# DecodeGenetics/BamQC

Measured on AMD Instinct MI355X. Metric: BAM records/sec (and GB/s vs HBM roofline), 150 bp PE, 1/2/4/8 MI355X, higher is better.
Workload: dtype u8/u32/u64 integer

## Files before the change

### bamqc_amd/csrc/k_short.hip

```cpp
#include "kernels_common.h"
#include "read_stats.h"
#include "swar.h"

#define KS_NH BQC_FAST_NH
#define KS_NB (8 * KS_NH)
#define KS_ND (2 * KS_NH)
#define KS_CSTRIDE (256 / KS_NB)
#define KS_LUTW (KS_NH == 2 ? 8 : 16)
#define KS_WAVES BQC_FAST_WAVES
#define KS_THREADS (KS_WAVES * 64)
#define KS_CT 256
#define KS_T8    0
#define KS_TRIP  (KS_T8 + 16384)
#define KS_CYC   (KS_TRIP + 1024)
#define KS_NC    (KS_CYC + 2 * 6 * KS_CT)
#define KS_GC    (KS_NC + 2 * (KS_CT + 1))
#define KS_AQ    (KS_GC + 2 * (KS_CT + 1))
#define KS_AC    (KS_AQ + 512)
#define KS_LUT   (KS_AC + 512)
#define KS_META  (KS_LUT + (KS_NB + 1) * KS_LUTW + (((KS_NB + 1) * KS_LUTW) % 4 ? 4 - ((KS_NB + 1) * KS_LUTW) % 4 : 0))
#define KS_MW    8
#define KS_RS    (KS_META + (KS_WAVES * 64 + 1) * KS_MW)
#define KS_WORDS (KS_RS + RS_WORDS)
#define KS_T8_PERIOD 16
#define KS_BIAS  512u

static_assert((KS_LUT % 4) == 0 && (KS_META % 4) == 0, "16-byte alignment of the LDS tables");

__device__ __forceinline__ bool t8_flush(uint32_t* lds, uint64_t* __restrict__ em, uint4* __restrict__ slot , uint32_t n_rows_used)
{
    if (slot && n_rows_used < BQC_T8_SPW) {
        uint4* row = slot + (size_t)n_rows_used * 4096u;
        uint4* src = (uint4*)(lds + KS_T8);
        for (uint32_t i = threadIdx.x; i < 4096u; i += blockDim.x) { row[i] = src[i]; src[i] = make_uint4(0, 0, 0, 0); }
        return true;
    }
    t8_atomics_out(lds + KS_T8, em);
    return false;
}

__device__ __forceinline__ uint32_t ks_trip_bin(uint32_t ix) { return ix ^ ((ix >> 2) & 0x11u); }
__device__ __forceinline__ uint32_t ks_trip_stream(uint32_t s) { return s ^ ((s >> 2) & 0x11111111u); }

__device__ __forceinline__ bool ks_flush(uint32_t* lds, const StateLayout& sl, uint64_t* __restrict__ state, uint32_t lane, uint4* __restrict__ slot, uint32_t n_rows_used)
{
    const uint64_t lb = sl.lane_base(lane);
    const bool wrote_row = t8_flush(lds, state + lb + sl.o_eightmer, slot, n_rows_used);
    for (uint32_t i = threadIdx.x; i < 1024; i += blockDim.x) {
        const uint32_t v = lds[KS_TRIP + i];
        if (!v) continue;
        lds[KS_TRIP + i] = 0;
        const uint32_t ix = ks_trip_bin(i);
        const uint32_t grp = i >> 8, f3 = (ix >> 6) & 3u, f2 = (ix >> 4) & 3u, f1 = (ix >> 2) & 3u, f0 = ix & 3u;
        uint32_t ctx, base;
        if (grp < 2u) { ctx = (f3 << 4) | (f2 << 2) | f0; base = f1; }
        else { ctx = ((3u - f0) << 4) | ((3u - f2) << 2) | (3u - f3); base = 3u - f1; }
        gadd(state + lb + sl.o_triplet + ctx * 16u + grp * 4u + base, v);
    }
    for (uint32_t i = threadIdx.x; i < 2 * 6 * KS_CT; i += blockDim.x) {
        const uint32_t v = lds[KS_CYC + i];
        if (!v) continue;
        lds[KS_CYC + i] = 0;
        const uint32_t m = i / (6 * KS_CT), c = (i / KS_CT) % 6, jj = i % KS_CT, j = (jj % KS_CSTRIDE) * KS_NB + jj / KS_CSTRIDE;
        if (j < sl.lcap) gadd(state + sl.mate_base(lane, m) + (c < 5 ? sl.m_dnacount + c * sl.lcap : sl.m_qualcount) + j, v);
    }
    for (uint32_t i = threadIdx.x; i < 2 * (KS_CT + 1); i += blockDim.x) {
        const uint32_t m = i / (KS_CT + 1), j = i % (KS_CT + 1);
        const uint64_t mb = sl.mate_base(lane, m);
        uint32_t v = lds[KS_NC + i];
        if (v && j <= sl.lcap) gadd(state + mb + sl.m_ncount + j, v);
        lds[KS_NC + i] = 0;
        v = lds[KS_GC + i];
        if (v && j <= sl.lcap) gadd(state + mb + sl.m_gccount + j, v);
        lds[KS_GC + i] = 0;
    }
    for (uint32_t i = threadIdx.x; i < 512; i += blockDim.x) {
        const uint64_t mb = sl.mate_base(lane, i >> 8);
        uint32_t v = lds[KS_AQ + i];
        if (v) gadd(state + mb + sl.m_avgqual + (i & 255), v);
        lds[KS_AQ + i] = 0;
        v = lds[KS_AC + i];
        if (v) gadd(state + mb + sl.m_avgceil + (i & 255), v);
        lds[KS_AC + i] = 0;
    }
    return wrote_row;
}

struct CycAcc {
    uint32_t l1[KS_NH][4];
    uint32_t qo[KS_ND], qe[KS_ND];
};
__device__ __forceinline__ void cyc_zero(CycAcc& A)
{
#pragma unroll
    for (int h = 0; h < KS_NH; ++h)
#pragma unroll
        for (int p = 0; p < 4; ++p) A.l1[h][p] = 0;
#pragma unroll
    for (int d = 0; d < KS_ND; ++d) { A.qo[d] = 0; A.qe[d] = 0; }
}
__device__ __noinline__ void cyc_spill_half(uint32_t a, uint32_t c, uint32_t g, uint32_t t, uint32_t* base )
{
    const uint32_t v[4] = {a, c, g, t};
#pragma unroll
    for (int p = 0; p < 4; ++p)
#pragma unroll
        for (int n = 0; n < 8; ++n) atomicAdd(base + p * KS_CT + KS_CSTRIDE * (7 - n), (v[p] >> (4 * n)) & 15u);
}
__device__ __noinline__ void cyc_qflush_pair(uint32_t o0, uint32_t e0, uint32_t o1, uint32_t e1, uint32_t* base )
{
    const uint32_t vo[2] = {o0, o1}, ve[2] = {e0, e1};
#pragma unroll
    for (int d = 0; d < 2; ++d) {
        atomicAdd(base + KS_CSTRIDE * (4 * d + 0), vo[d] >> 16);
        atomicAdd(base + KS_CSTRIDE * (4 * d + 1), ve[d] >> 16);
        atomicAdd(base + KS_CSTRIDE * (4 * d + 2), vo[d] & 0xFFFFu);
        atomicAdd(base + KS_CSTRIDE * (4 * d + 3), ve[d] & 0xFFFFu);
    }
}
__device__ __forceinline__ void cyc_spill(CycAcc& A, uint32_t* lds, uint32_t mate, uint32_t w)
{
#pragma unroll
    for (int h = 0; h < KS_NH; ++h) {
        cyc_spill_half(A.l1[h][0], A.l1[h][1], A.l1[h][2], A.l1[h][3], lds + KS_CYC + mate * 6 * KS_CT + w + KS_CSTRIDE * 8 * h);
#pragma unroll
        for (int p = 0; p < 4; ++p) A.l1[h][p] = 0;
    }
}
__device__ __forceinline__ void cyc_qflush(CycAcc& A, uint32_t* lds, uint32_t mate, uint32_t w)
{
#pragma unroll
    for (int h = 0; h < KS_NH; ++h) {
        cyc_qflush_pair(A.qo[2 * h], A.qe[2 * h], A.qo[2 * h + 1], A.qe[2 * h + 1], lds + KS_CYC + (mate * 6 + 5) * KS_CT + w + KS_CSTRIDE * 8 * h);
        A.qo[2 * h] = A.qe[2 * h] = A.qo[2 * h + 1] = A.qe[2 * h + 1] = 0;
    }
}
__device__ __forceinline__ void cyc_add(CycAcc& A, const Planes (&P)[KS_NH], const uint32_t (&Q)[KS_ND])
{
#pragma unroll
    for (int h = 0; h < KS_NH; ++h) { A.l1[h][0] += P[h].a; A.l1[h][1] += P[h].c; A.l1[h][2] += P[h].g; A.l1[h][3] += P[h].t; }
#pragma unroll
    for (int d = 0; d < KS_ND; ++d) { A.qe[d] += Q[d] & 0x00FF00FFu; A.qo[d] += __builtin_amdgcn_perm(0u, Q[d], 0x0C030C01u); }
}

#define KM_PRIM   0x10000u
#define KM_TRIP   0x20000u
#define KM_SEG    0x40000u

__device__ __forceinline__ void lut_nib(uint32_t (&d)[KS_NH], const uint32_t* e)
{
    if (KS_NH == 2) { const uint2 v = *(const uint2*)e; d[0] = v.x; d[1] = v.y; }
    else { const uint4 v = *(const uint4*)e; d[0] = v.x; d[1] = v.y; d[KS_NH - 2] = v.z; d[KS_NH - 1] = v.w; }
}
__device__ __forceinline__ void lut_byte(uint32_t (&d)[KS_ND], const uint32_t* e)
{
#pragma unroll
    for (int q = 0; q < KS_ND / 4; ++q) { const uint4 v = *(const uint4*)(e + 4 * q); d[4 * q] = v.x; d[4 * q + 1] = v.y; d[4 * q + 2] = v.z; d[4 * q + 3] = v.w; }
}

template <bool S> struct KsTile { static constexpr bool seg = S; };

struct Pre { uint32_t s[KS_NH + 1], q[KS_ND], e[KS_NH + 1]; uint32_t m0, pp, w5; };

__device__ __forceinline__ Pre ks_prefetch(const uint32_t* rec, uint32_t w, const uint8_t* seqb, const uint8_t* qualb)
{
    const uint4 ma = *(const uint4*)rec, mb = *(const uint4*)(rec + 4);
    const int32_t sw = (ma.x & 0x10u) ? -(int32_t)w : (int32_t)w;
    Pre P;
    P.m0 = ma.x;
    P.w5 = mb.y;
    P.pp = ma.w + (uint32_t)(KS_NB * sw);
    GVec<KS_NH + 1>::ldu(P.s, seqb + (uint32_t)(ma.y + (uint32_t)(KS_NB / 2 * sw)));
    GVec<KS_ND>::ldu(P.q, qualb + (uint32_t)(ma.z + (uint32_t)(KS_NB * sw)));
    const uint32_t* rn = (const uint32_t*)(uintptr_t)((uint64_t)mb.z | ((uint64_t)mb.w << 32));
    const int32_t di = min(max((int32_t)P.pp >> 3, 0), (int32_t)mb.x);
    GVec<KS_NH + 1>::lda(P.e, (const uint8_t*)(rn + di));
    return P;
}

__global__ __launch_bounds__(KS_THREADS) void k_short(DevBatch b, StateLayout sl, uint64_t* __restrict__ state, DevRefs refs,
                                                         uint32_t* __restrict__ err, uint32_t parts, uint4* __restrict__ t8rows,
                                                         uint32_t* __restrict__ t8_used, uint32_t t8_period)
{
    extern __shared__ uint32_t lds[];
    if ((uint32_t)(uintptr_t)(lds_u32*)lds != 0u) {
        if (threadIdx.x == 0) { atomicOr(err, BQC_DEVERR_INTERNAL); t8_used[blockIdx.x * BQC_T8_USED] = 0; }
        return;
    }
    for (uint32_t i = threadIdx.x; i < KS_WORDS; i += blockDim.x) lds[i] = 0;
    block_sync();
    const uint32_t M = 0x11111111u;
    const uint32_t ln = threadIdx.x & 63u, wave = (uint32_t)__builtin_amdgcn_readfirstlane((int)(threadIdx.x >> 6));
    const BatchDesc desc = *b.desc;
    const uint32_t W = desc.fast_w, rpw = 64u / W;
    const uint32_t slot = ln / W, w = ln % W, wnb = KS_NB * w;
    const bool lane_used = slot < rpw;
    const bool last_w = (w + 1u >= W) || ln == 63u;
    const uint32_t tile_cap = rpw * (64u / rpw);
    uint32_t* WM = lds + KS_META + wave * 64u * KS_MW;
    const uint32_t* DUMMY = lds + KS_META + KS_WAVES * 64u * KS_MW;
    const uint32_t* LUT = lds + KS_LUT;
    if (threadIdx.x <= KS_NB) {
        const uint32_t n = threadIdx.x;
        uint32_t* e = lds + KS_LUT + KS_LUTW * n;
        for (uint32_t h = 0; h < KS_NH; ++h) {
            const uint32_t v = n > 8u * h ? (n - 8u * h < 8u ? n - 8u * h : 8u) : 0u;
            e[h] = v ? 0xFFFFFFFFu << (4u * (8u - v)) : 0u;
        }
        for (uint32_t d = 0; d < KS_ND; ++d) {
            const uint32_t v = n > 4u * d ? (n - 4u * d < 4u ? n - 4u * d : 4u) : 0u;
            e[4 + d] = v ? 0xFFFFFFFFu << (8u * (4u - v)) : 0u;
        }
    }
    if (threadIdx.x < KS_MW) {
        const uint32_t t = threadIdx.x;
        lds[KS_META + KS_WAVES * 64u * KS_MW + t] = t == 1 || t == 2 ? KS_BIAS : t == 3 ? 8u * KS_NH - 1u : t == 5 ? (24u << 16) : t == 6 ? (uint32_t)(uintptr_t)state
                                   : t == 7 ? (uint32_t)((uintptr_t)state >> 32) : 0u;
    }
    block_sync();
    CycAcc A;
    cyc_zero(A);
    const uint32_t mate = slot < (rpw + 1u) / 2u ? 0u : 1u;
    uint32_t n1 = 0, n2 = 0;
    uint32_t cur_lane = 0xFFFFFFFFu, since_t8 = 0;
    uint4* const t8_slot = t8rows + (size_t)blockIdx.x * BQC_T8_SPW * 4096u;
    uint32_t t8_n = 0;
    T8Tags t8_tags;

    const uint8_t* g_seq = b.seq - KS_BIAS;
    const uint8_t* g_qual = b.qual - KS_BIAS;
    const uint32_t n_chunks = desc.n_chunks_fast;
    {
        const uint32_t cpw = (n_chunks + gridDim.x - 1) / gridDim.x;
        t8_period = max(t8_period, (cpw + BQC_T8_SPW - 2) / (BQC_T8_SPW - 1));
    }
    uint32_t ci = blockIdx.x, ci_step = gridDim.x, ci_end = n_chunks;
    if ((parts & 16u) && (gridDim.x & 7u) == 0u && n_chunks >= gridDim.x) {
        const uint32_t per = (n_chunks + 7u) >> 3, lo = (blockIdx.x & 7u) * per;
        ci = lo + (blockIdx.x >> 3); ci_step = gridDim.x >> 3; ci_end = min(n_chunks, lo + per);
    }
    for (;; ci += ci_step) {
        const bool done = ci >= ci_end;
        Chunk ch{0, 0, 0xFFFFFFFFu, 0, 0, 0, 0, 0};
        if (!done) ch = b.chunks_fast[ci];
        if (ch.lane != cur_lane) {
            if (cur_lane != 0xFFFFFFFFu) {
                if (lane_used) { cyc_spill(A, lds, mate, w); cyc_qflush(A, lds, mate, w); }
                n1 = n2 = 0;
                block_sync();
                if (ks_flush(lds, sl, state, cur_lane, t8_slot, t8_n)) { t8_tag(t8_tags, t8_n, cur_lane); ++t8_n; }
                rs_flush(lds + KS_RS, sl, state, cur_lane);
            }
            cur_lane = ch.lane;
            since_t8 = 0;
        }
        if (done) break;
        if (++since_t8 > t8_period) {
            since_t8 = 1;
            const bool to_row = t8_n < BQC_T8_SPW;
            uint32_t* row = (uint32_t*)(t8_slot + (size_t)t8_n * 4096u);
            uint64_t* emf = state + sl.lane_base(cur_lane) + sl.o_eightmer;
#pragma unroll 4
            for (uint32_t k = 0; k < 16384u / (KS_WAVES * 64u); ++k) {
                const uint32_t i = (wave * (16384u / (KS_WAVES * 64u)) + k) * 64u + ln;
                const uint32_t v = atomicExch(&lds[KS_T8 + i], 0u);
                if (to_row) row[i] = v;
                else if (v) {
#pragma unroll
                    for (uint32_t b8 = 0; b8 < 4; ++b8)
                        if ((v >> (8u * b8)) & 0xFFu) gadd(emf + 4u * i + ((4u - b8) & 3u), (v >> (8u * b8)) & 0xFFu);
                }
            }
            if (to_row) { t8_tag(t8_tags, t8_n, cur_lane); ++t8_n; }
        }
        const uint64_t lb = sl.lane_base(cur_lane);
        uint64_t* em = state + lb + sl.o_eightmer;
        const uint32_t n_seg = ch.count - ch.aux;
        const uint32_t my_tiles = ch.aux > wave * tile_cap ? (ch.aux - wave * tile_cap + KS_WAVES * tile_cap - 1u) / (KS_WAVES * tile_cap) : 0u;
        const uint32_t sw0 = (wave + KS_WAVES - ci % KS_WAVES) % KS_WAVES;
        const uint32_t seg_tiles = n_seg > sw0 * tile_cap ? (n_seg - sw0 * tile_cap + KS_WAVES * tile_cap - 1u) / (KS_WAVES * tile_cap) : 0u;
        for (uint32_t tix = 0; tix < my_tiles + seg_tiles; ++tix) {
        const bool seg_tile = tix >= my_tiles;
        const uint32_t tb = seg_tile ? (sw0 + (tix - my_tiles) * KS_WAVES) * tile_cap : (wave + tix * KS_WAVES) * tile_cap;
        const uint32_t p_first = seg_tile ? ch.aux : 0u, p_n = seg_tile ? n_seg : ch.aux;
        const uint32_t tn = min(tile_cap, p_n - tb);
        __builtin_amdgcn_s_setprio(3);
        uint32_t r;
        bool stat;
        {
            const uint32_t t = ch.first + p_first + tb + ln;
            r = ln < tn ? b.perm[t] : 0xFFFFFFFFu;
            const bool live = r != 0xFFFFFFFFu;
            const bool seg = live && (r & BQC_ENTRY_SEG);
            stat = live && !seg;
            TripSeg sg{0, 0, 0, 0};
            if (seg) { sg = b.segs[r & ~BQC_ENTRY_SEG]; r = sg.r; }
            uint4 R0 = make_uint4(0u, KS_BIAS, KS_BIAS, 8u * KS_NH - 1u);
            uint4 R1 = make_uint4(0u, 24u << 16, (uint32_t)(uintptr_t)state, (uint32_t)((uintptr_t)state >> 32));
            if (live) {
                const uint32_t fl = b.flag[r];
                R0.x = fl & 0xFFFFu;
                if (!(fl & 0x900u) && (fl & 0xC0u)) {
                    const uint32_t L = b.l_seq[r];
                    const bool rc = fl & 0x10u, noq = fl & BQC_FLAG_NO_QUAL;
                    const int32_t o0 = rc ? (int32_t)L - KS_NB : 0;
                    R0.x |= (seg ? KM_SEG : KM_PRIM) | (L << 20);
                    R0.y = b.seq_off[r] + (uint32_t)((o0 - 1) >> 1) + KS_BIAS;
                    R0.z = (noq ? 0u : b.qual_off[r]) + (uint32_t)o0 + KS_BIAS;
                    R1.y = ((o0 & 1) ? 28u : 24u) << 16;
                    const int32_t rid = b.rid[r];
                    if ((fl & BQC_FLAG_TRIPLET) && b.n_cigar[r] >= 1 && L >= 3 && !noq && rid >= 0 && (uint32_t)rid < refs.n_refs &&
                        refs.refn[rid] != nullptr) {
                        const int64_t pos = seg ? (int64_t)sg.posv : (int64_t)b.pos[r];
                        const int64_t reflen = (int64_t)refs.len[rid];
                        int64_t ia = 1, ib = (int64_t)L - 1;
                        if (seg) { ia = sg.range & 0xFFu; ib = (sg.range >> 8) & 0xFFu; }
                        else {
                            const uint32_t n0 = b.cigar[b.cigar_off[r]] >> 4;
                            if (n0 != 0u && (int64_t)n0 < ib) ib = n0;
                        }
                        if (1 - pos > ia) ia = 1 - pos;
                        if (reflen - 1 - pos < ib) ib = reflen - 1 - pos;
                        if (ib > ia && pos > -(1 << 30) && pos < (1 << 30)) {
                            const uint32_t ja = rc ? L - (uint32_t)ib : (uint32_t)ia, jb = rc ? L - (uint32_t)ia : (uint32_t)ib;
                            const uint64_t nd8 = (uint64_t)(reflen + 7) >> 3;
                            R0.x |= KM_TRIP;
                            R0.w = (uint32_t)((int32_t)pos + o0 + 8 * KS_NH - 1);
                            R1.x = (uint32_t)(nd8 + KS_NH - 1);
                            R1.y |= ja | (jb << 8);
                            const uint64_t rn = (uint64_t)(uintptr_t)refs.refn[rid];
                            R1.z = (uint32_t)rn; R1.w = (uint32_t)(rn >> 32);
                        }
                    }
                }
            }
            uint4* Mr = (uint4*)(WM + ln * KS_MW);
            Mr[0] = R0; Mr[1] = R1;
        }
        asm volatile("" ::: "memory");
        __builtin_amdgcn_wave_barrier();
        const uint32_t n_groups = tn / rpw;
        Pre cur = ks_prefetch(lane_used ? WM + slot * KS_MW : DUMMY, w, g_seq, g_qual);
        if ((parts & 8u) && __ballot(stat)) read_stats(b, sl, state, refs, err, lds + KS_RS, stat ? r : 0u, stat, stat);
        __builtin_amdgcn_s_setprio(0);
        auto groups = [&](auto tile_kind) __attribute__((always_inline)) {
        constexpr bool SEG = decltype(tile_kind)::seg;
        for (uint32_t g = 0; g < n_groups; ++g) {
            const uint32_t k = g * rpw + slot;
            const uint32_t m0 = cur.m0, w5 = cur.w5, L = (m0 >> 20) & 0xFFu;
            const bool rc = m0 & 0x10u;
            const uint32_t nv = (uint32_t)min(max((int32_t)L - (int32_t)wnb, 0), KS_NB);
            const uint32_t nvq = (m0 & BQC_FLAG_NO_QUAL) ? 0u : nv;
            uint32_t xm[KS_NH], qm[KS_ND];
            lut_nib(xm, LUT + KS_LUTW * nv);
            lut_byte(qm, LUT + KS_LUTW * nvq + 4u);
            uint32_t X[KS_NH];
            {
                const uint32_t sh = w5 >> 16;
                uint32_t bs[KS_NH + 1], F[KS_NH];
#pragma unroll
                for (int h = 0; h <= KS_NH; ++h) bs[h] = bswap32(cur.s[h]);
#pragma unroll
                for (int h = 0; h < KS_NH; ++h) F[h] = alignbit(bs[h], bs[h + 1], sh);
#pragma unroll
                for (int h = 0; h < KS_NH; ++h)
                    X[h] = (rc ? __brev(F[KS_NH - 1 - h]) : F[h]) & xm[h];
            }
            uint32_t Q[KS_ND];
            {
                const uint32_t sel = rc ? 0x07060504u : 0x00010203u;
                uint32_t any = 0;
#pragma unroll
                for (int d = 0; d < KS_ND; ++d) { Q[d] = vperm(cur.q[KS_ND - 1 - d], cur.q[d], sel) & qm[d]; any |= Q[d]; }
                if (any & 0x80808080u) {
                    bool bad = false;
#pragma unroll
                    for (int d = 0; d < KS_ND; ++d)
#pragma unroll
                        for (int k8 = 0; k8 < 4; ++k8) bad |= ((Q[d] >> (8 * k8)) & 0xFFu) > 222u;
                    if (bad) atomicOr(err, BQC_DEVERR_QUAL);
                }
            }
            uint32_t E[KS_NH];
            {
                const uint32_t sh = 28u - 4u * (cur.pp & 7u);
                uint32_t F[KS_NH];
#pragma unroll
                for (int h = 0; h < KS_NH; ++h) F[h] = alignbit(cur.e[h], cur.e[h + 1], sh);
#pragma unroll
                for (int h = 0; h < KS_NH; ++h) E[h] = rc ? __brev(F[KS_NH - 1 - h]) : F[h];
            }
            {
                cur = ks_prefetch(lane_used && g + 1u < n_groups ? WM + (k + rpw) * KS_MW : DUMMY, w, g_seq, g_qual);
            }
            Planes P[KS_NH];
#pragma unroll
            for (int h = 0; h < KS_NH; ++h) P[h] = planes_of(X[h]);
            if ((parts & 1u) && !SEG) {
                cyc_add(A, P, Q);
                if (++n1 == 15u) { if (lane_used) cyc_spill(A, lds, mate, w); n1 = 0; }
                if (++n2 == 255u) { if (lane_used) cyc_qflush(A, lds, mate, w); n2 = 0; }
                uint32_t oth[KS_NH], oany = 0;
#pragma unroll
                for (int h = 0; h < KS_NH; ++h) { oth[h] = xm[h] & M & ~P[h].oh; oany |= oth[h]; }
                if (oany) {
                    uint32_t* ob = lds + KS_CYC + (mate * 6 + 4) * KS_CT + w;
#pragma unroll
                    for (int h = 0; h < KS_NH; ++h) {
                        uint32_t o = oth[h];
                        while (o) { const uint32_t bit = (uint32_t)__ffs((int)o) - 1u; o &= o - 1u; atomicAdd(ob + KS_CSTRIDE * (8u * h + 7u - (bit >> 2)), 1u); }
                    }
                }
                uint32_t v = 0, vn = 0, vgc = 0;
#pragma unroll
                for (int d = 0; d < KS_ND; ++d) v = __builtin_amdgcn_sad_u8(Q[d], 0u, v);
#pragma unroll
                for (int h = 0; h < KS_NH; ++h) { vn += (uint32_t)__popc(P[h].n); vgc += (uint32_t)__popc(P[h].c | P[h].g); }
                v |= vn << 16;
                v += vgc << 24;
                if (lane_used) {
                    uint32_t* sw = WM + k * KS_MW + 1;
                    if (w == 0u) *sw = 0u;
                    atomicAdd(sw, v);
                }
            }
            uint32_t cn[KS_NH], nb[KS_NH + 1];
#pragma unroll
            for (int h = 0; h < KS_NH; ++h) {
                cn[h] = (P[h].c | P[h].t) | ((P[h].g | P[h].t) << 1);
                nb[h] = P[h].n | (~xm[h] & M);
            }
            if ((parts & 2u) && !SEG) {
                uint32_t S[KS_NH / 2 + 1];
#pragma unroll
                for (int j = 0; j < KS_NH / 2; ++j) S[j] = vperm(squeeze2(cn[2 * j]), squeeze2(cn[2 * j + 1]), 0x05040100u);
                S[KS_NH / 2] = lane_next(S[0]);
                nb[KS_NH] = lane_next(nb[0]);
                if (last_w) nb[KS_NH] = M;
                uint32_t f[KS_NH];
                {
                    uint32_t sa[KS_NH + 1], sb[KS_NH + 1];
#pragma unroll
                    for (int h = 0; h < KS_NH; ++h) sa[h] = nb[h] | alignbit(nb[h], nb[h + 1], 28);
                    sa[KS_NH] = nb[KS_NH] | (nb[KS_NH] << 4);
#pragma unroll
                    for (int h = 0; h < KS_NH; ++h) sb[h] = sa[h] | alignbit(sa[h], sa[h + 1], 24);
                    sb[KS_NH] = sa[KS_NH] | (sa[KS_NH] << 8);
#pragma unroll
                    for (int h = 0; h < KS_NH; ++h) f[h] = ~(sb[h] | alignbit(sb[h], sb[h + 1], 16));
                }
#pragma unroll
                for (int j = 0; j < KS_NH / 2; ++j) {
                    if (nv > 16u * j) {
                        const uint32_t c32 = S[j], cx = S[j + 1];
                        uint32_t old[16];
#pragma unroll
                        for (int kw = 0; kw < 16; ++kw) {
                            const uint32_t h = kw < 8 ? c32 >> (16 - 2 * kw) : kw == 8 ? c32 : alignbit(c32, cx, 48 - 2 * kw);
                            const uint32_t one = bfe(f[2 * j + (kw >> 3)], 28 - 4 * (kw & 7), 1);
                            old[kw] = __hip_atomic_fetch_add(lds_at(h & 0xFFFCu), alignbyte(one, one, h), __ATOMIC_RELAXED, __HIP_MEMORY_SCOPE_WORKGROUP);
                        }
                        uint32_t hot0 = 0, hot1 = 0;
#pragma unroll
                        for (int kk = 0; kk < 8; ++kk) { hot0 |= old[kk]; hot1 |= old[8 + kk]; }
                        if (hot0 & 0x80808080u)
                            t8_check<0>(em, c32, cx, f[2 * j], old[0], old[1], old[2], old[3], old[4], old[5], old[6], old[7]);
                        if (hot1 & 0x80808080u)
                            t8_check<8>(em, c32, cx, f[2 * j + 1], old[8], old[9], old[10], old[11], old[12], old[13], old[14], old[15]);
                    }
                }
            }
            if ((parts & 4u) && __ballot(m0 & KM_TRIP)) {
                const uint32_t rcm = rc ? 0x33333333u : 0u;
                uint32_t I[KS_NH + 2], bad[KS_NH + 2];
#pragma unroll
                for (int h = 0; h < KS_NH; ++h) {
                    const uint32_t x = ~P[h].oh & M;
                    const uint32_t ct = cn[h] | ((x | (x << 1)) & rcm);
                    I[h + 1] = (E[h] & 0xCCCCCCCCu) | ct;
                    const uint32_t t = I[h + 1] ^ (I[h + 1] >> 2);
                    bad[h + 1] = ((t | (t >> 1)) & M) | nb[h];
                }
                bad[0] = lane_prev(bad[KS_NH]); bad[KS_NH + 1] = lane_next(bad[1]);
                I[0] = lane_prev(I[KS_NH]); I[KS_NH + 1] = lane_next(I[1]);
                const uint32_t ja = (uint32_t)min(max((int32_t)(w5 & 0xFFu) - (int32_t)wnb, 0), KS_NB);
                const uint32_t jb = (uint32_t)min(max((int32_t)((w5 >> 8) & 0xFFu) - (int32_t)wnb, 0), KS_NB);
                uint32_t pa[KS_NH], pb[KS_NH];
                lut_nib(pa, LUT + KS_LUTW * ja);
                lut_nib(pb, LUT + KS_LUTW * jb);
                uint32_t qf[KS_ND];
#pragma unroll
                for (int d = 0; d < KS_ND; ++d) {
                    const uint32_t x = Q[d] & 0x7F7F7F7Fu;
                    const uint32_t fq = (x + 0x6C6C6C6Cu) & ~(x + 0x21212121u) & ~Q[d];
                    const uint32_t y = fq & 0x80808080u;
                    qf[d] = y | (y << 4);
                }
                uint32_t ok[KS_NH], okany = 0;
#pragma unroll
                for (int h = 0; h < KS_NH; ++h) {
                    const uint32_t fl = alignbit(bad[h], bad[h + 1], 4) | alignbit(bad[h + 1], bad[h + 2], 28);
                    ok[h] = P[h].oh & ~fl & pb[h] & ~pa[h] & (vperm(qf[2 * h], qf[2 * h + 1], 0x07050301u) >> 3);
                    okany |= ok[h];
                }
                if (okany) {
                    uint32_t* tbin = lds + KS_TRIP + ((rc ? 2u : 0u) + ((m0 & 0x40u) ? 0u : 1u)) * 256u;
#pragma unroll
                    for (int h = 0; h < KS_NH; ++h) {
                        if (!ok[h]) continue;
                        const uint32_t SA = ks_trip_stream(alignbit(I[h], I[h + 1], 6)), SB = ks_trip_stream(alignbit(I[h + 1], I[h + 2], 22));
#pragma unroll
                        for (int t = 0; t < 8; ++t) {
                            const uint32_t ix = t < 6 ? bfe(SA, 20 - 4 * t, 8) : bfe(SB, 12 - 4 * (t - 6), 8);
                            atomicAdd(tbin + ix, bfe(ok[h], 28 - 4 * t, 1));
                        }
                    }
                }
            }
        }
        };
        if (seg_tile) groups(KsTile<true>{}); else groups(KsTile<false>{});
        asm volatile("" ::: "memory");
        __builtin_amdgcn_wave_barrier();
        if ((parts & 1u) && ln < tn) {
            const uint32_t m0 = WM[ln * KS_MW];
            if (m0 & KM_PRIM) {
                const uint32_t L = (m0 >> 20) & 0xFFu, sum = WM[ln * KS_MW + 1];
                const uint32_t qs = sum & 0xFFFFu, nN = (sum >> 16) & 0xFFu, nGC = sum >> 24, rm = (m0 & 0x40u) ? 0u : 1u;
                atomicAdd(&lds[KS_NC + rm * (KS_CT + 1) + nN], 1u);
                atomicAdd(&lds[KS_GC + rm * (KS_CT + 1) + nGC], 1u);
                if (L > 0) {
                    atomicAdd(&lds[KS_AQ + rm * 256 + (small_div(2u * qs + L, 2u * L) & 255u)], 1u);
                    atomicAdd(&lds[KS_AC + rm * 256 + (small_div(qs + L - 1u, L) & 255u)], 1u);
                }
            }
        }
        asm volatile("" ::: "memory");
        __builtin_amdgcn_wave_barrier();
        }
    }
    if (threadIdx.x == 0) t8_directory(t8_used + blockIdx.x * BQC_T8_USED, t8_n, t8_tags);
}


__global__ void k_ref_nibbles(const uint8_t* __restrict__ dna5, uint64_t len, uint32_t* __restrict__ out, uint64_t nd8)
{
    const uint64_t d = (uint64_t)blockIdx.x * blockDim.x + threadIdx.x;
    if (d >= nd8 + 2 * KS_NH) return;
    uint32_t v = 0;
    if (d >= KS_NH)
        for (uint32_t t = 0; t < 8; ++t) {
            const uint64_t p = (d - KS_NH) * 8 + t;
            if (p < len) {
                const uint32_t r = dna5[p] & 3u;
                v |= ((r << 2) | ((~r & 1u) << 1) | ((~r >> 1) & 1u)) << (28u - 4u * t);
            }
        }
    out[d] = v;
}

extern "C" void bqc_launch_ref_nibbles(const uint8_t* dna5, uint64_t len, uint32_t* out, uint64_t nd8, hipStream_t s)
{
    hipLaunchKernelGGL(k_ref_nibbles, dim3((uint32_t)((nd8 + 2 * KS_NH + 255) / 256)), dim3(256), 0, s, dna5, len, out, nd8);
}

extern "C" uint32_t bqc_short_parts()
{
    static uint32_t parts = 0xFFFFFFFFu;
    if (parts == 0xFFFFFFFFu) {
        const char* e = getenv("BQC_SHORT_PARTS");
        parts = e ? (uint32_t)atoi(e) : 15u;
        const char* x = getenv("BQC_SHORT_XCD");
        if (x && atoi(x) != 0) parts |= 16u;
    }
    return parts;
}

extern "C" hipError_t bqc_short_init()
{
    return hipFuncSetAttribute(reinterpret_cast<const void*>(&k_short), hipFuncAttributeMaxDynamicSharedMemorySize, KS_WORDS * 4);
}

__global__ __launch_bounds__(256) void k_t8_fold(const uint32_t* __restrict__ rows, const uint32_t* __restrict__ used, uint32_t n_slots,
                                                    uint64_t* __restrict__ em, uint32_t lane)
{
    const uint32_t i = blockIdx.x * blockDim.x + threadIdx.x;
    uint32_t A = 0, B = 0, C = 0, D = 0;
    const uint32_t s0 = blockIdx.y * 64u, s1 = min(n_slots, s0 + 64u);
    for (uint32_t sidx = s0; sidx < s1; ++sidx) {
        const uint32_t n = min(used[sidx * BQC_T8_USED], (uint32_t)BQC_T8_SPW);
        const uint64_t tags = (uint64_t)used[sidx * BQC_T8_USED + 1] | ((uint64_t)used[sidx * BQC_T8_USED + 2] << 32);
        const uint32_t* slot = rows + (size_t)sidx * BQC_T8_SPW * 16384u + i;
        uint32_t v[BQC_T8_SPW];
#pragma unroll
        for (uint32_t f = 0; f < BQC_T8_SPW; ++f) v[f] = f < n && ((uint32_t)(tags >> (8u * f)) & 0xFFu) == lane ? slot[(size_t)f * 16384u] : 0u;
#pragma unroll
        for (uint32_t f = 0; f < BQC_T8_SPW; ++f) { A += v[f] & 0xFFu; B += (v[f] >> 8) & 0xFFu; C += (v[f] >> 16) & 0xFFu; D += v[f] >> 24; }
    }
    if (A) gadd(em + 4u * i + 0u, A);
    if (B) gadd(em + 4u * i + 3u, B);
    if (C) gadd(em + 4u * i + 2u, C);
    if (D) gadd(em + 4u * i + 1u, D);
}

extern "C" void bqc_launch_short(const DevBatch& b, const StateLayout& sl, uint64_t* state, const DevRefs& refs, uint32_t* err,
                                 uint32_t grid, uint32_t* t8rows, uint32_t* t8_used, hipStream_t s)
{
    if (grid == 0) return;
    static const hipError_t attr_once = bqc_short_init();
    (void)attr_once;
    static uint32_t env_period = 0xFFFFFFFFu;
    if (env_period == 0xFFFFFFFFu) { const char* e = getenv("BQC_T8_PERIOD"); env_period = e && atoi(e) > 0 ? (uint32_t)atoi(e) : 0u; }
    hipLaunchKernelGGL(k_short, dim3(grid), dim3(KS_THREADS), KS_WORDS * 4, s, b, sl, state, refs, err, bqc_short_parts(), (uint4*)t8rows, t8_used,
                       env_period ? env_period : KS_T8_PERIOD);
}

extern "C" void bqc_launch_t8_fold(const uint32_t* t8rows, const uint32_t* t8_used, uint32_t n_slots, const StateLayout& sl, uint64_t* state, uint32_t lane,
                                   hipStream_t s)
{
    if (!n_slots) return;
    hipLaunchKernelGGL(k_t8_fold, dim3(64, (n_slots + 63) / 64), dim3(256), 0, s, t8rows, t8_used, n_slots, state + sl.lane_base(lane) + sl.o_eightmer, lane);
}
```

Measured before the change: 4.431 billion.

## Split leftover chunks across idle blocks, inline spill helpers, hoist cycle spill checks

Forces the per-cycle spill and quality flush helpers to be inlined rather than called. Chunks left over after an even division across the grid are now shared: several blocks each take a slice of a leftover chunk's groups, so blocks are not idle during the tail. The per-group spill counters are replaced by an inner run loop that stops at the next spill boundary, which takes the counter checks off the per-group path. The 8-mer atomic block is now gated by the flag mask rather than the valid length. Inlining raises register pressure, and the tail split adds bookkeeping.

```diff
diff --git a/bamqc_amd/csrc/k_short.hip b/bamqc_amd/csrc/k_short.hip
--- a/bamqc_amd/csrc/k_short.hip
+++ b/bamqc_amd/csrc/k_short.hip
@@ -99,7 +99,7 @@
 #pragma unroll
     for (int d = 0; d < KS_ND; ++d) { A.qo[d] = 0; A.qe[d] = 0; }
 }
-__device__ __noinline__ void cyc_spill_half(uint32_t a, uint32_t c, uint32_t g, uint32_t t, uint32_t* base )
+__device__ __forceinline__ void cyc_spill_half(uint32_t a, uint32_t c, uint32_t g, uint32_t t, uint32_t* base )
 {
     const uint32_t v[4] = {a, c, g, t};
 #pragma unroll
@@ -107,7 +107,7 @@
 #pragma unroll
         for (int n = 0; n < 8; ++n) atomicAdd(base + p * KS_CT + KS_CSTRIDE * (7 - n), (v[p] >> (4 * n)) & 15u);
 }
-__device__ __noinline__ void cyc_qflush_pair(uint32_t o0, uint32_t e0, uint32_t o1, uint32_t e1, uint32_t* base )
+__device__ __forceinline__ void cyc_qflush_pair(uint32_t o0, uint32_t e0, uint32_t o1, uint32_t e1, uint32_t* base )
 {
     const uint32_t vo[2] = {o0, o1}, ve[2] = {e0, e1};
 #pragma unroll
@@ -235,14 +235,24 @@
         t8_period = max(t8_period, (cpw + BQC_T8_SPW - 2) / (BQC_T8_SPW - 1));
     }
     uint32_t ci = blockIdx.x, ci_step = gridDim.x, ci_end = n_chunks;
+    uint32_t left_ci = 0xFFFFFFFFu, left_j = 0, left_split = 1;
     if ((parts & 16u) && (gridDim.x & 7u) == 0u && n_chunks >= gridDim.x) {
         const uint32_t per = (n_chunks + 7u) >> 3, lo = (blockIdx.x & 7u) * per;
         ci = lo + (blockIdx.x >> 3); ci_step = gridDim.x >> 3; ci_end = min(n_chunks, lo + per);
+    } else {
+        const uint32_t n_full = n_chunks / gridDim.x * gridDim.x, n_left = n_chunks - n_full;
+        ci_end = n_full;
+        if (n_left) {
+            left_split = min(gridDim.x / n_left, tile_cap / rpw);
+            if (blockIdx.x < n_left * left_split) { left_ci = n_full + blockIdx.x % n_left; left_j = blockIdx.x / n_left; }
+        }
     }
     for (;; ci += ci_step) {
-        const bool done = ci >= ci_end;
+        uint32_t cidx = ci, part_j = 0, part_n = 1;
+        bool done = ci >= ci_end;
+        if (done && left_ci != 0xFFFFFFFFu) { cidx = left_ci; part_j = left_j; part_n = left_split; left_ci = 0xFFFFFFFFu; done = false; }
         Chunk ch{0, 0, 0xFFFFFFFFu, 0, 0, 0, 0, 0};
-        if (!done) ch = b.chunks_fast[ci];
+        if (!done) ch = b.chunks_fast[cidx];
         if (ch.lane != cur_lane) {
             if (cur_lane != 0xFFFFFFFFu) {
                 if (lane_used) { cyc_spill(A, lds, mate, w); cyc_qflush(A, lds, mate, w); }
@@ -277,13 +287,18 @@
         uint64_t* em = state + lb + sl.o_eightmer;
         const uint32_t n_seg = ch.count - ch.aux;
         const uint32_t my_tiles = ch.aux > wave * tile_cap ? (ch.aux - wave * tile_cap + KS_WAVES * tile_cap - 1u) / (KS_WAVES * tile_cap) : 0u;
-        const uint32_t sw0 = (wave + KS_WAVES - ci % KS_WAVES) % KS_WAVES;
+        const uint32_t sw0 = (wave + KS_WAVES - cidx % KS_WAVES) % KS_WAVES;
         const uint32_t seg_tiles = n_seg > sw0 * tile_cap ? (n_seg - sw0 * tile_cap + KS_WAVES * tile_cap - 1u) / (KS_WAVES * tile_cap) : 0u;
         for (uint32_t tix = 0; tix < my_tiles + seg_tiles; ++tix) {
         const bool seg_tile = tix >= my_tiles;
-        const uint32_t tb = seg_tile ? (sw0 + (tix - my_tiles) * KS_WAVES) * tile_cap : (wave + tix * KS_WAVES) * tile_cap;
+        uint32_t tb = seg_tile ? (sw0 + (tix - my_tiles) * KS_WAVES) * tile_cap : (wave + tix * KS_WAVES) * tile_cap;
         const uint32_t p_first = seg_tile ? ch.aux : 0u, p_n = seg_tile ? n_seg : ch.aux;
-        const uint32_t tn = min(tile_cap, p_n - tb);
+        uint32_t tn = min(tile_cap, p_n - tb);
+        if (part_n > 1u) {
+            const uint32_t t = tn / rpw, g0 = part_j * t / part_n, g1 = (part_j + 1u) * t / part_n;
+            tb += g0 * rpw; tn = (g1 - g0) * rpw;
+            if (!tn) continue;
+        }
         __builtin_amdgcn_s_setprio(3);
         uint32_t r;
         bool stat;
@@ -345,7 +360,10 @@
         __builtin_amdgcn_s_setprio(0);
         auto groups = [&](auto tile_kind) __attribute__((always_inline)) {
         constexpr bool SEG = decltype(tile_kind)::seg;
-        for (uint32_t g = 0; g < n_groups; ++g) {
+        for (uint32_t g = 0; g < n_groups;) {
+        const bool cyc = (parts & 1u) && !SEG;
+        const uint32_t run = cyc ? min(n_groups - g, min(15u - n1, 255u - n2)) : n_groups - g;
+        for (const uint32_t g_end = g + run; g < g_end; ++g) {
             const uint32_t k = g * rpw + slot;
             const uint32_t m0 = cur.m0, w5 = cur.w5, L = (m0 >> 20) & 0xFFu;
             const bool rc = m0 & 0x10u;
@@ -398,8 +416,6 @@
             for (int h = 0; h < KS_NH; ++h) P[h] = planes_of(X[h]);
             if ((parts & 1u) && !SEG) {
                 cyc_add(A, P, Q);
-                if (++n1 == 15u) { if (lane_used) cyc_spill(A, lds, mate, w); n1 = 0; }
-                if (++n2 == 255u) { if (lane_used) cyc_qflush(A, lds, mate, w); n2 = 0; }
                 uint32_t oth[KS_NH], oany = 0;
 #pragma unroll
                 for (int h = 0; h < KS_NH; ++h) { oth[h] = xm[h] & M & ~P[h].oh; oany |= oth[h]; }
@@ -451,7 +467,7 @@
                 }
 #pragma unroll
                 for (int j = 0; j < KS_NH / 2; ++j) {
-                    if (nv > 16u * j) {
+                    if ((f[2 * j] | f[2 * j + 1]) & M) {
                         const uint32_t c32 = S[j], cx = S[j + 1];
                         uint32_t old[16];
 #pragma unroll
@@ -517,6 +533,11 @@
                     }
                 }
             }
+        }
+        if (cyc) {
+            if ((n1 += run) == 15u) { if (lane_used) cyc_spill(A, lds, mate, w); n1 = 0; }
+            if ((n2 += run) == 255u) { if (lane_used) cyc_qflush(A, lds, mate, w); n2 = 0; }
+        }
         }
         };
         if (seg_tile) groups(KsTile<true>{}); else groups(KsTile<false>{});
```

Result: faster. 4.476 billion, median of 6 (+1.0%).
